# camlab-ethz/poseidon

Measured on AMD Instinct MI355X. Metric: PDE-grid samples/sec (fwd+bwd), higher is better.
Workload: dtype fp16

## Files before the change

### poseidon_amd/csrc/block_fused.h

```cpp
#pragma once
#include "common.h"

template <int C> struct KPitch { static constexpr int KP = (C + 31) / 32 * 32, P = KP + 8; };

struct ClnRowsOut {
  const float* bias;
  void* z; int z_dt;
  float* mean; float* rstd;
  const float* time; const float* gw_w; const float* gw_b; const float* bw_w; const float* bw_b; const float* sscale;
  const float* resid;
  float* out; bf16_t* out16;
  int M, rows_per_sample;
  float eps;
};

template <int C, int TT>
__device__ __forceinline__ void cln_rows_epilogue(f32x4_t (&Y)[TT][C / 16], float* patch_base, int row0, const ClnRowsOut& p,
                                                  bf16_t* tile16 = nullptr) {
  constexpr int KJ = (C + 31) / 32, NT = C / 16, CP = C + 4;
  constexpr bool RAG = (C % 32) != 0;
  static_assert(C % 16 == 0, "channel tiles");
  const int lane = threadIdx.x & 63, wave = threadIdx.x >> 6, g = lane >> 4, lc = lane & 15;
  float* Ct = patch_base + wave * 16 * CP;
  const int prow = lane >> 2, q = lane & 3;
#pragma unroll
  for (int tt = 0; tt < TT; ++tt) {
#pragma unroll
    for (int nt = 0; nt < NT; ++nt)
#pragma unroll
      for (int r = 0; r < 4; ++r) Ct[(g * 4 + r) * CP + nt * 16 + lc] = Y[tt][nt][r];
    __builtin_amdgcn_wave_barrier();
    const int grow = row0 + tt * 16 + prow;
    const bool valid = grow < p.M;
    float v[KJ][8];
    float s1 = 0.f;
#pragma unroll
    for (int pp = 0; pp < KJ; ++pp) {
      const int col = pp * 32 + q * 8;
      const bool pv = !RAG || col < C;
#pragma unroll
      for (int j = 0; j < 8; ++j) v[pp][j] = 0.f;
      if (pv) {
        const float4 x0 = *(const float4*)(Ct + prow * CP + col), x1 = *(const float4*)(Ct + prow * CP + col + 4);
        float bb[8];
        ld8(p.bias, SCOT_F32, col, bb);
        v[pp][0] = x0.x + bb[0]; v[pp][1] = x0.y + bb[1]; v[pp][2] = x0.z + bb[2]; v[pp][3] = x0.w + bb[3];
        v[pp][4] = x1.x + bb[4]; v[pp][5] = x1.y + bb[5]; v[pp][6] = x1.z + bb[6]; v[pp][7] = x1.w + bb[7];
      }
#pragma unroll
      for (int j = 0; j < 8; ++j) s1 += v[pp][j];
    }
    s1 += __shfl_xor(s1, 1, 64); s1 += __shfl_xor(s1, 2, 64);
    const float mean = s1 * (1.0f / C);
    float s2 = 0.f;
#pragma unroll
    for (int pp = 0; pp < KJ; ++pp) {
      if (RAG && pp * 32 + q * 8 >= C) continue;
#pragma unroll
      for (int j = 0; j < 8; ++j) { const float d = v[pp][j] - mean; s2 += d * d; }
    }
    s2 += __shfl_xor(s2, 1, 64); s2 += __shfl_xor(s2, 2, 64);
    const float rstd = 1.0f / sqrtf(s2 * (1.0f / C) + p.eps);
    if (valid) {
      const size_t base = (size_t)grow * C;
      if (p.mean && q == 0) { p.mean[grow] = mean; p.rstd[grow] = rstd; }
      const int samp = grow / p.rows_per_sample;
      const float t = p.time ? p.time[samp] : 0.f;
      const float sc = p.sscale ? p.sscale[samp] : 1.f;
#pragma unroll
      for (int pp = 0; pp < KJ; ++pp) {
        const int col = pp * 32 + q * 8;
        if (RAG && col >= C) continue;
        if (p.z) st8(p.z, p.z_dt, base + col, v[pp]);
        float gw[8], gb[8], bw[8], bbv[8], res[8], o[8];
        ld8(p.gw_b, SCOT_F32, col, gb); ld8(p.bw_b, SCOT_F32, col, bbv);
        if (p.gw_w) { ld8(p.gw_w, SCOT_F32, col, gw); ld8(p.bw_w, SCOT_F32, col, bw); }
        ld8(p.resid, SCOT_F32, base + col, res);
#pragma unroll
        for (int j = 0; j < 8; ++j) {
          const float ga = p.gw_w ? gw[j] * t + gb[j] : gb[j];
          const float be = p.gw_w ? bw[j] * t + bbv[j] : bbv[j];
          o[j] = sc * (ga * ((v[pp][j] - mean) * rstd) + be) + res[j];
        }
        st8(p.out, SCOT_F32, base + col, o);
        if (p.out16) st8(p.out16, SCOT_BF16, base + col, o);
        if (tile16) store8_ct(tile16 + (tt * 16 + prow) * (C + 8) + col, o);
      }
    } else if (tile16) {
      const float zero[8] = {0.f, 0.f, 0.f, 0.f, 0.f, 0.f, 0.f, 0.f};
#pragma unroll
      for (int pp = 0; pp < KJ; ++pp)
        if (!RAG || pp * 32 + q * 8 < C) store8_ct(tile16 + (tt * 16 + prow) * (C + 8) + pp * 32 + q * 8, zero);
    }
    __builtin_amdgcn_wave_barrier();
  }
}

struct ClnRowsBwd {
  const float* g;
  const void* z; int z_dt; const float* mean; const float* rstd;
  const float* time; const float* gw_w; const float* gw_b; const float* sscale;
  bf16_t* dz;
  float* d_gw_w; float* d_gw_b; float* d_bw_w; float* d_bw_b;
  float* partial;
  int M, rows_per_sample;
};

template <int C> struct ClnBwdLds {
// ... 130 lines not shown
```

### poseidon_amd/csrc/mlp_fused.hip

```cpp
#include "common.h"
#include <stdlib.h>

#include "block_fused.h"

typedef unsigned int u32x4_t __attribute__((ext_vector_type(4)));

struct MlpArgs {
  const bf16_t* h16; const float* h;
  const bf16_t* W1; const float* b1;
  const bf16_t* W2; const float* b2;
  float* out; bf16_t* out16;
  bf16_t* act; bf16_t* dact;
  void* z; int z_dt; float* mean; float* rstd;
  const float* time; const float* gw_w; const float* gw_b; const float* bw_w; const float* bw_b; const float* sscale;
  int M, rows_per_sample, hid;
  float eps;
};

template <int C, int HC> struct MlpFwdLds {
  static constexpr size_t WBYTES = (size_t)(HC * KPitch<C>::P + C * (HC + 8)) * 2 + (size_t)256 * 4, PBYTES = (size_t)4 * 16 * (C + 4) * 4;
  static constexpr size_t bytes = WBYTES > PBYTES ? WBYTES : PBYTES;
};

template <int C, int HC, int TT, bool HTILE>
__device__ __forceinline__ void mlp_fwd_body(const MlpArgs& p, char* smem, const bf16_t* htile, bf16_t* otile = nullptr) {
  constexpr bool RAG = (C % 32) != 0;
  constexpr int KJ = (C + 31) / 32;
  constexpr int NT = C / 16;
  constexpr int NB = HC / 32;
  constexpr int P1 = KPitch<C>::P;
  constexpr int P2 = HC + 8;
  constexpr int CP = C + 4;
  constexpr int W1_EL = HC * P1, W2_EL = C * P2;
  constexpr int N1 = HC * C / 8, N2 = C * HC / 8;
  constexpr int PW1 = (N1 + 255) / 256, PW2 = (N2 + 255) / 256;
  static_assert(RAG || (N1 % 256 == 0 && N2 % 256 == 0), "weight chunk pieces must divide over the 256 threads");
  static_assert(HC <= 256 && C % 16 == 0 && HC % 32 == 0 && (W1_EL * 2) % 16 == 0 && ((W1_EL + W2_EL) * 2) % 16 == 0, "layout");
  bf16_t* W1c = (bf16_t*)smem;
  bf16_t* W2c = W1c + W1_EL;
  float* b1c = (float*)(W2c + W2_EL);

  const int tid = threadIdx.x, lane = tid & 63, wave = tid >> 6, g = lane >> 4, lc = lane & 15;
  const int HID = p.hid, nch = HID / HC;
  const int row0 = (blockIdx.x * 4 + wave) * (16 * TT);

  Frag<bf16_t> hf[TT][KJ];
#pragma unroll
  for (int tt = 0; tt < TT; ++tt) {
// ... 39 lines not shown
      *(u32x4_t*)(W1c + rho * P1 + k8) = r1[u];
    }
#pragma unroll
    for (int u = 0; u < PW2; ++u) {
      const int i = tid + u * 256;
      if (RAG && i >= N2) continue;
      const int row = i / (HC / 8), c8 = (i % (HC / 8)) * 8;
      *(u32x4_t*)(W2c + row * P2 + c8) = r2[u];
    }
    b1c[tid] = rb1;
    if (RAG) {
      constexpr int PADP = (KPitch<C>::KP - C) / 8;
      const u32x4_t z = {0u, 0u, 0u, 0u};
      for (int i = tid; i < HC * PADP; i += 256) *(u32x4_t*)(W1c + (i / PADP) * P1 + C + (i % PADP) * 8) = z;
    }
  };

  f32x4_t Y[TT][NT];
#pragma unroll
  for (int tt = 0; tt < TT; ++tt)
#pragma unroll
    for (int nt = 0; nt < NT; ++nt) Y[tt][nt] = (f32x4_t){0.f, 0.f, 0.f, 0.f};

  load_chunk(0);
  store_chunk();
  __syncthreads();

  auto multiply_chunk = [&](int c) {
#pragma unroll
    for (int blk = 0; blk < NB; ++blk) {
      f32x4_t U[TT][2];
#pragma unroll
      for (int tt = 0; tt < TT; ++tt) { U[tt][0] = (f32x4_t){0.f, 0.f, 0.f, 0.f}; U[tt][1] = (f32x4_t){0.f, 0.f, 0.f, 0.f}; }
#pragma unroll
      for (int j = 0; j < KJ; ++j) {
#pragma unroll
        for (int t = 0; t < 2; ++t) {
          const Frag<bf16_t> w = lds_frag_kc(W1c, P1, blk * 32 + t * 16, j * 32, lane);
#pragma unroll
          for (int tt = 0; tt < TT; ++tt) mma16(U[tt][t], w, hf[tt][j]);
        }
      }
      const float4 ba = *(const float4*)(b1c + blk * 32 + g * 8), bb = *(const float4*)(b1c + blk * 32 + g * 8 + 4);
      const float bias[8] = {ba.x, ba.y, ba.z, ba.w, bb.x, bb.y, bb.z, bb.w};
      Frag<bf16_t> af[TT];
#pragma unroll
      for (int tt = 0; tt < TT; ++tt) {
        float av[8], dv[8];
#pragma unroll
        for (int t = 0; t < 2; ++t)
#pragma unroll
          for (int r = 0; r < 4; ++r) {
            const float x = U[tt][t][r] + bias[4 * t + r];
            float cdf, e;
            gelu_terms(x, cdf, e);
            av[4 * t + r] = x * cdf;
            dv[4 * t + r] = cdf + x * 0.3989422804014327f * e;
          }
        af[tt] = frag_from_f32<bf16_t>(av);
        if (p.act || p.dact) {
          const int row = row0 + tt * 16 + lc;
          if (row < p.M) {
            const size_t o = (size_t)row * HID + (size_t)c * HC + blk * 32 + g * 8;
            if (p.act) *(s16x8_t*)(p.act + o) = af[tt].v;
            if (p.dact) *(s16x8_t*)(p.dact + o) = frag_from_f32<bf16_t>(dv).v;
          }
        }
      }
#pragma unroll
      for (int nt = 0; nt < NT; ++nt) {
        const Frag<bf16_t> w = lds_frag_kc(W2c, P2, nt * 16, blk * 32, lane);
#pragma unroll
        for (int tt = 0; tt < TT; ++tt) mma16(Y[tt][nt], af[tt], w);
      }
    }
  };
  for (int c = 0; c + 1 < nch; ++c) {
    load_chunk(c + 1);
    multiply_chunk(c);
    __syncthreads();
    store_chunk();
    __syncthreads();
  }
  multiply_chunk(nch - 1);
  __syncthreads();

  ClnRowsOut e;
  e.bias = p.b2; e.z = p.z; e.z_dt = p.z_dt; e.mean = p.mean; e.rstd = p.rstd; e.time = p.time; e.gw_w = p.gw_w; e.gw_b = p.gw_b; e.bw_w = p.bw_w;
  e.bw_b = p.bw_b; e.sscale = p.sscale; e.resid = p.h; e.out = p.out; e.out16 = p.out16; e.M = p.M; e.rows_per_sample = p.rows_per_sample;
  e.eps = p.eps;
  cln_rows_epilogue<C, TT>(Y, (float*)smem, row0, e, otile);
}

template <int C, int HC, int TT>
__global__ __launch_bounds__(256, 2) void mlp_fused_kernel(MlpArgs p) {
  __shared__ __attribute__((aligned(16))) char smem[MlpFwdLds<C, HC>::bytes];
  mlp_fwd_body<C, HC, TT, false>(p, smem, nullptr);
}

static int mlp_chunk(int) { return 64; }

template <int C, int HC, int TT>
static int launch_mlp(const MlpArgs& a, hipStream_t s) {
  static_assert((HC * C / 8) % 256 == 0, "ragged weight chunk");
  const int rows_per_wg = 64 * TT;
  dim3 grid((a.M + rows_per_wg - 1) / rows_per_wg), block(256);
  hipLaunchKernelGGL((mlp_fused_kernel<C, HC, TT>), grid, block, 0, s, a);
  return scot_check_launch();
}

static int scot_mlp_tt_override() {
  static int tt_env = -1;
  if (tt_env < 0) { const char* e = getenv("SCOT_MLP_TT"); tt_env = e ? atoi(e) : 0; }
  return tt_env;
}

extern "C" int scot_mlp_block_fwd(const void* h16, const float* h, const void* W1, const float* b1, const void* W2, const float* b2,
                                  float* out, void* out16, void* act, void* dact, float* z, float* mean, float* rstd,
                                  const float* time, const float* gw_w, const float* gw_b, const float* bw_w, const float* bw_b,
                                  const float* sample_scale, int M, int rows_per_sample, int C, int hid, float eps,
// ... 59 lines not shown
  static constexpr size_t htile_bytes(int TT) { return (size_t)64 * TT * (C + 8) * 2; }
};

template <int C, int HC, int TT, bool KEEP, bool GIN = false, bool RECOMP = false>
__device__ __forceinline__ void mlp_bwd_body(const MlpBwdArgs& p, char* smem, float (*gkeep)[(C + 31) / 32][8],
                                             const float (*gin)[(C + 31) / 32][8] = nullptr) {
  constexpr bool RAG = (C % 32) != 0;
  constexpr int KJ = (C + 31) / 32, NT = C / 16, NB = HC / 32;
  constexpr int P1 = C + 8;
  constexpr int P2 = HC + 8;
  constexpr int CP = C + 4;
  constexpr int W1_EL = HC * P1, W2_EL = C * P2;
  constexpr int N1 = HC * C / 8, N2 = C * HC / 8;
  constexpr int PW1 = (N1 + 255) / 256, PW2 = (N2 + 255) / 256;
  static_assert((W1_EL * 2) % 16 == 0, "layout");
  static_assert(RAG || (N1 % 256 == 0 && N2 % 256 == 0), "weight chunk pieces must divide over the 256 threads");
  static_assert(!RAG || !RECOMP, "the recomputing form reads W1 K-contiguously: C % 32 == 0 only");
  bf16_t* W1c = (bf16_t*)smem;
  bf16_t* W2c = W1c + W1_EL;
  const int tid = threadIdx.x, lane = tid & 63, wave = tid >> 6, g = lane >> 4, lc = lane & 15;
  const int HID = p.hid, nch = HID / HC;
  const int wg_row0 = blockIdx.x * (64 * TT);
  const int row0 = wg_row0 + wave * (16 * TT);
  const int prow = lane >> 2, q = lane & 3;

  u32x4_t r1[PW1], r2[PW2];
  auto load_chunk = [&](int c) {
    const bf16_t* s1 = p.W1 + (size_t)c * HC * C;
#pragma unroll
    for (int u = 0; u < PW1; ++u) {
      const int i = min(tid + u * 256, N1 - 1);
      r1[u] = *(const u32x4_t*)(s1 + (size_t)i * 8);
    }
#pragma unroll
    for (int u = 0; u < PW2; ++u) {
      const int i = min(tid + u * 256, N2 - 1);
      const int row = i / (HC / 8), c8 = (i % (HC / 8)) * 8;
      r2[u] = *(const u32x4_t*)(p.W2 + (size_t)row * HID + (size_t)c * HC + c8);
    }
  };
  auto store_chunk = [&]() {
#pragma unroll
    for (int u = 0; u < PW1; ++u) {
      const int i = tid + u * 256;
      if (RAG && i >= N1) continue;
      *(u32x4_t*)(W1c + (i / (C / 8)) * P1 + (i % (C / 8)) * 8) = r1[u];
    }
// ... 115 lines not shown
        asm volatile("" ::"v"(af[tt].v));
#else
        if (p.du && rowt[tt] < p.M) *(s16x8_t*)(p.du + (size_t)rowt[tt] * HID + (size_t)c * HC + blk * 32 + g * 8) = af[tt].v;
#endif
      }
#pragma unroll
      for (int nt = 0; nt < NT; ++nt) {
        const Frag<bf16_t> w = lds_frag_ks(W1c, P1, nt * 16, blk * 32 + g * 8, blk * 32 + g * 8 + 4, lane, p.use_tr);
#pragma unroll
        for (int tt = 0; tt < TT; ++tt) mma16(Y[tt][nt], af[tt], w);
      }
    }
  };
  for (int c = 0; c + 1 < nch; ++c) {
    load_chunk(c + 1);
    multiply_chunk(c);
    __syncthreads();
    store_chunk();
    __syncthreads();
  }
  multiply_chunk(nch - 1);
  __syncthreads();

  float* Ct = (float*)smem + wave * 16 * CP;
#pragma unroll
  for (int tt = 0; tt < TT; ++tt) {
#pragma unroll
    for (int nt = 0; nt < NT; ++nt)
#pragma unroll
      for (int r = 0; r < 4; ++r) Ct[(g * 4 + r) * CP + nt * 16 + lc] = Y[tt][nt][r];
    __builtin_amdgcn_wave_barrier();
    const int grow = row0 + tt * 16 + prow;
    if (grow < p.M) {
      const size_t base = (size_t)grow * C;
#pragma unroll
      for (int pp = 0; pp < KJ; ++pp) {
        const int col = pp * 32 + q * 8;
        if (RAG && col >= C) {
          if (KEEP) {
#pragma unroll
            for (int j = 0; j < 8; ++j) gkeep[tt][pp][j] = 0.f;
          }
          continue;
        }
        const float4 x0 = *(const float4*)(Ct + prow * CP + col), x1 = *(const float4*)(Ct + prow * CP + col + 4);
        float gi[8], o[8];
        ld8(p.g, SCOT_F32, base + col, gi);
        o[0] = gi[0] + x0.x; o[1] = gi[1] + x0.y; o[2] = gi[2] + x0.z; o[3] = gi[3] + x0.w;
        o[4] = gi[4] + x1.x; o[5] = gi[5] + x1.y; o[6] = gi[6] + x1.z; o[7] = gi[7] + x1.w;
        st8(p.g_out, SCOT_F32, base + col, o);
        if (KEEP) {
#pragma unroll
          for (int j = 0; j < 8; ++j) gkeep[tt][pp][j] = o[j];
        }
      }
    } else if (KEEP) {
#pragma unroll
      for (int pp = 0; pp < KJ; ++pp)
#pragma unroll
        for (int j = 0; j < 8; ++j) gkeep[tt][pp][j] = 0.f;
    }
    __builtin_amdgcn_wave_barrier();
  }
}

template <int C, int HC, int TT>
__global__ __launch_bounds__(256, 2) void mlp_bwd_fused_kernel(MlpBwdArgs p) {
  __shared__ __attribute__((aligned(16))) char smem[MlpBwdLds<C, HC>::bytes];
  mlp_bwd_body<C, HC, TT, false>(p, smem, nullptr);
}

extern int g_scot_use_tr;
// ... 22 lines not shown
  if (rows_per_sample % 64 != 0) return SCOT_ERR_UNSUPPORTED;
  MlpBwdArgs a;
  a.g = g; a.g_out = g_out; a.z = z; a.z_dt = SCOT_F32; a.mean = mean; a.rstd = rstd; a.time = time; a.gw_w = gw_w; a.gw_b = gw_b; a.sscale = sample_scale;
  a.partial = nullptr; a.h16 = nullptr; a.b1 = nullptr;
  a.dact = (const bf16_t*)dact; a.W1 = (const bf16_t*)W1; a.W2 = (const bf16_t*)W2; a.dz = (bf16_t*)dz; a.du = (bf16_t*)du;
  a.d_gw_w = d_gw_w; a.d_gw_b = d_gw_b; a.d_bw_w = d_bw_w; a.d_bw_b = d_bw_b;
  a.M = M; a.rows_per_sample = rows_per_sample; a.hid = hid; a.use_tr = g_scot_use_tr;
  if (C == 96) {
    return tt == 2 ? launch_mlp_bwd<96, 64, 2>(a, stream) : launch_mlp_bwd<96, 64, 1>(a, stream);
  }
  return tt == 2 ? launch_mlp_bwd<192, 64, 2>(a, stream) : launch_mlp_bwd<192, 64, 1>(a, stream);
}

struct ProjClnArgs {
  const bf16_t* a; const bf16_t* W;
  ClnRowsOut e;
};

template <int C> struct ProjFwdLds {
  static constexpr size_t WBYTES = (size_t)C * (96 + 8) * 2, PBYTES = (size_t)4 * 16 * (C + 4) * 4;
  static constexpr size_t bytes = WBYTES > PBYTES ? WBYTES : PBYTES;
};

template <int C, int TT>
__device__ __forceinline__ void proj_cln_fwd_body(const ProjClnArgs& p, char* smem, bf16_t* tile16) {
  constexpr bool RAG = (C % 32) != 0;
  constexpr int KJ = (C + 31) / 32, NT = C / 16, KC = RAG ? KJ * 32 : 96, NKC = RAG ? 1 : C / KC;
  constexpr int KCR = RAG ? C : KC;
  constexpr int PW = KC + 8;
  constexpr int NP = C * KCR / 8, PWN = (NP + 255) / 256;
  static_assert(RAG || C % KC == 0, "K chunking");
  bf16_t* Wc = (bf16_t*)smem;
  const int tid = threadIdx.x, lane = tid & 63, wave = tid >> 6, g = lane >> 4, lc = lane & 15;
  const int row0 = (blockIdx.x * 4 + wave) * (16 * TT);

  Frag<bf16_t> af[TT][KJ];
#pragma unroll
  for (int tt = 0; tt < TT; ++tt) {
    const bf16_t* src = p.a + (size_t)min(row0 + tt * 16 + lc, p.e.M - 1) * C + g * 8;
    const s16x8_t zero8 = {0, 0, 0, 0, 0, 0, 0, 0};
#pragma unroll
    for (int j = 0; j < KJ; ++j) af[tt][j].v = (!RAG || j * 32 + g * 8 < C) ? *(const s16x8_t*)(src + j * 32) : zero8;
  }
  f32x4_t Y[TT][NT];
#pragma unroll
  for (int tt = 0; tt < TT; ++tt)
#pragma unroll
    for (int nt = 0; nt < NT; ++nt) Y[tt][nt] = (f32x4_t){0.f, 0.f, 0.f, 0.f};
  u32x4_t rw[PWN];
#pragma unroll
  for (int kc = 0; kc < NKC; ++kc) {
#pragma unroll
    for (int u = 0; u < PWN; ++u) {
      const int i = min(tid + u * 256, NP - 1);
      rw[u] = *(const u32x4_t*)(p.W + (size_t)(i / (KCR / 8)) * C + kc * KC + (i % (KCR / 8)) * 8);
    }
    if (kc) __syncthreads();
#pragma unroll
    for (int u = 0; u < PWN; ++u) {
      const int i = tid + u * 256;
      if (i < NP) *(u32x4_t*)(Wc + (i / (KCR / 8)) * PW + (i % (KCR / 8)) * 8) = rw[u];
    }
    if (RAG) {
      constexpr int PADP = (KC - KCR) / 8;
      const u32x4_t z = {0u, 0u, 0u, 0u};
      for (int i = tid; i < C * PADP; i += 256) *(u32x4_t*)(Wc + (i / PADP) * PW + KCR + (i % PADP) * 8) = z;
    }
    __syncthreads();
#pragma unroll
    for (int j = 0; j < KC / 32; ++j)
#pragma unroll
      for (int nt = 0; nt < NT; ++nt) {
        const Frag<bf16_t> w = lds_frag_kc(Wc, PW, nt * 16, j * 32, lane);
#pragma unroll
        for (int tt = 0; tt < TT; ++tt) mma16(Y[tt][nt], af[tt][kc * (KC / 32) + j], w);
      }
  }
  __syncthreads();
  cln_rows_epilogue<C, TT>(Y, (float*)smem, row0, p.e, tile16);
}

template <int C, int TT>
__global__ __launch_bounds__(256, 2) void proj_cln_fused_kernel(ProjClnArgs p) {
  __shared__ __attribute__((aligned(16))) char smem[ProjFwdLds<C>::bytes];
  proj_cln_fwd_body<C, TT>(p, smem, nullptr);
}

struct TailFwdArgs {
  ProjClnArgs pj; MlpArgs m;
  const bf16_t* Wqkv; const float* bqkv; bf16_t* qkv;
};

template <int C> struct QkvEpi {
  static constexpr int NC = (3 * C) % 96 == 0 ? 96 : 48;
  static constexpr size_t bytes = (size_t)NC * KPitch<C>::P * 2 + (size_t)4 * 16 * (NC + 4) * 4;
};
template <int C, int TT>
__device__ __forceinline__ void qkv_epilogue(const bf16_t* tile, const bf16_t* Wqkv, const float* bqkv, bf16_t* qkv, int M, char* smem) {
  constexpr bool RAG = (C % 32) != 0;
  constexpr int KJ = (C + 31) / 32, NC = QkvEpi<C>::NC, NCH = 3 * C / NC;
  constexpr int PW = KPitch<C>::P, NP = NC * C / 8, PWN = (NP + 255) / 256, CP = NC + 4;
  static_assert((3 * C) % NC == 0 && NC % 16 == 0, "qkv column chunks");
  const int tid = threadIdx.x, lane = tid & 63, wave = tid >> 6, g = lane >> 4, lc = lane & 15;
  const int row0 = (blockIdx.x * 4 + wave) * (16 * TT);
  Frag<bf16_t> af[TT][KJ];
#pragma unroll
  for (int tt = 0; tt < TT; ++tt)
#pragma unroll
    for (int j = 0; j < KJ; ++j) {
      const s16x8_t zero8 = {0, 0, 0, 0, 0, 0, 0, 0};
      af[tt][j].v = (!RAG || j * 32 + g * 8 < C) ? *(const s16x8_t*)(tile + (tt * 16 + lc) * (C + 8) + j * 32 + g * 8) : zero8;
    }
  bf16_t* Wc = (bf16_t*)smem;
  float* Ct = (float*)(smem + (size_t)NC * PW * 2) + wave * 16 * CP;
  const int prow = lane >> 2, q = lane & 3;
  u32x4_t rw[PWN];
#pragma unroll 1
  for (int nc = 0; nc < NCH; ++nc) {
    const bf16_t* src = Wqkv + (size_t)nc * NC * C;
#pragma unroll
    for (int u = 0; u < PWN; ++u) rw[u] = *(const u32x4_t*)(src + (size_t)min(tid + u * 256, NP - 1) * 8);
    __syncthreads();
#pragma unroll
    for (int u = 0; u < PWN; ++u) {
      const int i = tid + u * 256;
      if (i < NP) *(u32x4_t*)(Wc + (i / (C / 8)) * PW + (i % (C / 8)) * 8) = rw[u];
    }
    if (RAG) {
      constexpr int PADP = (KPitch<C>::KP - C) / 8;
      const u32x4_t z = {0u, 0u, 0u, 0u};
      for (int i = tid; i < NC * PADP; i += 256) *(u32x4_t*)(Wc + (i / PADP) * PW + C + (i % PADP) * 8) = z;
    }
    __syncthreads();
    f32x4_t Y[TT][NC / 16];
#pragma unroll
    for (int tt = 0; tt < TT; ++tt)
#pragma unroll
      for (int nt = 0; nt < NC / 16; ++nt) Y[tt][nt] = (f32x4_t){0.f, 0.f, 0.f, 0.f};
#pragma unroll
    for (int j = 0; j < KJ; ++j)
#pragma unroll
      for (int nt = 0; nt < NC / 16; ++nt) {
        const Frag<bf16_t> w = lds_frag_kc(Wc, PW, nt * 16, j * 32, lane);
#pragma unroll
        for (int tt = 0; tt < TT; ++tt) mma16(Y[tt][nt], af[tt][j], w);
      }
#pragma unroll
    for (int tt = 0; tt < TT; ++tt) {
#pragma unroll
      for (int nt = 0; nt < NC / 16; ++nt)
#pragma unroll
        for (int r = 0; r < 4; ++r) Ct[(g * 4 + r) * CP + nt * 16 + lc] = Y[tt][nt][r];
      __builtin_amdgcn_wave_barrier();
      const int grow = row0 + tt * 16 + prow;
      if (grow < M) {
#pragma unroll
        for (int pp = 0; pp < (NC + 31) / 32; ++pp) {
          const int col = pp * 32 + q * 8;
          if (NC % 32 != 0 && col >= NC) continue;
          const float4 x0 = *(const float4*)(Ct + prow * CP + col), x1 = *(const float4*)(Ct + prow * CP + col + 4);
          float o[8] = {x0.x, x0.y, x0.z, x0.w, x1.x, x1.y, x1.z, x1.w};
          if (bqkv) {
            float bb[8];
            ld8(bqkv, SCOT_F32, nc * NC + col, bb);
#pragma unroll
            for (int j = 0; j < 8; ++j) o[j] += bb[j];
          }
          st8(qkv, SCOT_BF16, (size_t)grow * (3 * C) + nc * NC + col, o);
        }
      }
      __builtin_amdgcn_wave_barrier();
    }
  }
}

template <int C, int HC, int TT, bool QKV>
__global__ __launch_bounds__(256, 2) void tail_fwd_fused_kernel(TailFwdArgs p) {
  constexpr size_t PATCH = (size_t)4 * 16 * (C + 4) * 4, TILE = (size_t)4 * 16 * TT * (C + 8) * 2;
  constexpr size_t A = ProjFwdLds<C>::bytes > PATCH + TILE ? ProjFwdLds<C>::bytes : PATCH + TILE;
  constexpr size_t QB = QkvEpi<C>::bytes;
  constexpr size_t B = A > MlpFwdLds<C, HC>::bytes ? A : MlpFwdLds<C, HC>::bytes;
  constexpr size_t LDS = (QKV && QB > B) ? QB : B;
  __shared__ __attribute__((aligned(16))) char smem[LDS];
  bf16_t* tile = (bf16_t*)(smem + PATCH) + (threadIdx.x >> 6) * 16 * TT * (C + 8);
  proj_cln_fwd_body<C, TT>(p.pj, smem, tile);
  __builtin_amdgcn_wave_barrier();
  mlp_fwd_body<C, HC, TT, true>(p.m, smem, tile, QKV ? tile : nullptr);
  if (QKV) {
    __builtin_amdgcn_wave_barrier();
    qkv_epilogue<C, TT>(tile, p.Wqkv, p.bqkv, p.qkv, p.m.M, smem);
  }
}

template <int C, int HC, int TT>
static int launch_tail_fwd(const TailFwdArgs& a, hipStream_t s) {
  dim3 grid((a.m.M + 64 * TT - 1) / (64 * TT)), block(256);
  if (a.qkv) hipLaunchKernelGGL((tail_fwd_fused_kernel<C, HC, TT, true>), grid, block, 0, s, a);
  else hipLaunchKernelGGL((tail_fwd_fused_kernel<C, HC, TT, false>), grid, block, 0, s, a);
  return scot_check_launch();
}

struct ProjClnBwdArgs {
  const bf16_t* W;
  bf16_t* da;
  ClnRowsBwd b;
  int use_tr;
};

template <int C> struct ProjBwdLds {
  static constexpr size_t WBYTES = (size_t)96 * (C + 8) * 2, PBYTES = (size_t)4 * 16 * (C + 4) * 4, P1BYTES = ClnBwdLds<C>::bytes;
  static constexpr size_t bytes = WBYTES > PBYTES ? (WBYTES > P1BYTES ? WBYTES : P1BYTES) : (PBYTES > P1BYTES ? PBYTES : P1BYTES);
};

template <int C, int TT, bool GREG>
__device__ __forceinline__ void proj_cln_bwd_body(const ProjClnBwdArgs& p, char* smem, const float (*greg)[(C + 31) / 32][8]) {
  constexpr bool RAG = (C % 32) != 0;
  constexpr int NT = C / 16, KC = RAG ? KPitch<C>::KP : 96, NKC = RAG ? 1 : C / KC;
  constexpr int KCR = RAG ? C : KC;
  constexpr int PW = C + 8;
  constexpr int NP = KCR * C / 8, PWN = (NP + 255) / 256;
  constexpr int CP = C + 4;
// ... 51 lines not shown
      for (int pp = 0; pp < (C + 31) / 32; ++pp) {
        const int col = pp * 32 + q * 8;
        if (RAG && col >= C) continue;
        const float4 x0 = *(const float4*)(Ct + prow * CP + col), x1 = *(const float4*)(Ct + prow * CP + col + 4);
        const float o[8] = {x0.x, x0.y, x0.z, x0.w, x1.x, x1.y, x1.z, x1.w};
        st8(p.da, SCOT_BF16, (size_t)grow * C + col, o);
      }
    }
    __builtin_amdgcn_wave_barrier();
  }
}

template <int C, int TT>
__global__ __launch_bounds__(256, 2) void proj_cln_bwd_fused_kernel(ProjClnBwdArgs p) {
  __shared__ __attribute__((aligned(16))) char smem[ProjBwdLds<C>::bytes];
  proj_cln_bwd_body<C, TT, false>(p, smem, nullptr);
}

struct TailBwdArgs {
  MlpBwdArgs m; ProjClnBwdArgs pj;
  const bf16_t* dqkv; const bf16_t* Wqkv;
};

template <int C, int TT>
__device__ __forceinline__ void qkv_dgrad_prologue(const bf16_t* dqkv, const bf16_t* Wqkv, float* gio, int M, char* smem, int use_tr,
                                                   float (*gk)[C / 32][8]) {
  constexpr int K3 = 3 * C, NT = C / 16, KC = 96, NKC = K3 / KC;
  constexpr int PW = C + 8, NP = KC * C / 8, PWN = (NP + 255) / 256, CP = C + 4;
  bf16_t* Wc = (bf16_t*)smem;
  const int tid = threadIdx.x, lane = tid & 63, wave = tid >> 6, g = lane >> 4, lc = lane & 15;
  const int row0 = (blockIdx.x * 4 + wave) * (16 * TT);
  f32x4_t Y[TT][NT];
#pragma unroll
  for (int tt = 0; tt < TT; ++tt)
#pragma unroll
    for (int nt = 0; nt < NT; ++nt) Y[tt][nt] = (f32x4_t){0.f, 0.f, 0.f, 0.f};
  u32x4_t rw[PWN];
#pragma unroll
  for (int kc = 0; kc < NKC; ++kc) {
    const bf16_t* src = Wqkv + (size_t)kc * KC * C;
#pragma unroll
    for (int u = 0; u < PWN; ++u) rw[u] = *(const u32x4_t*)(src + (size_t)min(tid + u * 256, NP - 1) * 8);
    Frag<bf16_t> af[TT][KC / 32];
#pragma unroll
    for (int tt = 0; tt < TT; ++tt) {
      const bf16_t* arow = dqkv + (size_t)min(row0 + tt * 16 + lc, M - 1) * K3 + kc * KC + g * 8;
#pragma unroll
// ... 4 lines not shown
    for (int u = 0; u < PWN; ++u) {
      const int i = tid + u * 256;
      if (i < NP) *(u32x4_t*)(Wc + (i / (C / 8)) * PW + (i % (C / 8)) * 8) = rw[u];
    }
    __syncthreads();
#pragma unroll
    for (int j = 0; j < KC / 32; ++j)
#pragma unroll
      for (int nt = 0; nt < NT; ++nt) {
        const Frag<bf16_t> w = lds_frag_ks(Wc, PW, nt * 16, j * 32 + g * 8, j * 32 + g * 8 + 4, lane, use_tr);
#pragma unroll
        for (int tt = 0; tt < TT; ++tt) mma16(Y[tt][nt], af[tt][j], w);
      }
  }
  __syncthreads();
  float* Ct = (float*)smem + wave * 16 * CP;
  const int prow = lane >> 2, q = lane & 3;
#pragma unroll
  for (int tt = 0; tt < TT; ++tt) {
#pragma unroll
    for (int nt = 0; nt < NT; ++nt)
#pragma unroll
      for (int r = 0; r < 4; ++r) Ct[(g * 4 + r) * CP + nt * 16 + lc] = Y[tt][nt][r];
    __builtin_amdgcn_wave_barrier();
    const int grow = row0 + tt * 16 + prow;
#pragma unroll
    for (int pp = 0; pp < C / 32; ++pp) {
      const int col = pp * 32 + q * 8;
      if (grow < M) {
        const float4 x0 = *(const float4*)(Ct + prow * CP + col), x1 = *(const float4*)(Ct + prow * CP + col + 4);
        float gi[8];
        ld8(gio, SCOT_F32, (size_t)grow * C + col, gi);
        gi[0] += x0.x; gi[1] += x0.y; gi[2] += x0.z; gi[3] += x0.w; gi[4] += x1.x; gi[5] += x1.y; gi[6] += x1.z; gi[7] += x1.w;
        st8(gio, SCOT_F32, (size_t)grow * C + col, gi);
#pragma unroll
        for (int j = 0; j < 8; ++j) gk[tt][pp][j] = gi[j];
      } else {
#pragma unroll
        for (int j = 0; j < 8; ++j) gk[tt][pp][j] = 0.f;
      }
    }
    __builtin_amdgcn_wave_barrier();
  }
}

template <int C, int HC, int TT, bool PRO, bool RECOMP>
__global__ __launch_bounds__(256, 2) void tail_bwd_fused_kernel(TailBwdArgs p) {
  constexpr size_t L0 = MlpBwdLds<C, HC>::bytes > ProjBwdLds<C>::bytes ? MlpBwdLds<C, HC>::bytes : ProjBwdLds<C>::bytes;
  constexpr size_t L1 = MlpBwdLds<C, HC>::bytes + (RECOMP ? MlpBwdLds<C, HC>::htile_bytes(TT) : 0);
  constexpr size_t LDS = L0 > L1 ? L0 : L1;
  __shared__ __attribute__((aligned(16))) char smem[LDS];
  float gk[TT][(C + 31) / 32][8];
  if constexpr (PRO) {
    static_assert(C % 32 == 0, "the qkv-dgrad prologue exists for C % 32 == 0 only");
    qkv_dgrad_prologue<C, TT>(p.dqkv, p.Wqkv, (float*)p.m.g, p.m.M, smem, p.m.use_tr, gk);
    __syncthreads();
    if (C <= 96 && !RECOMP) mlp_bwd_body<C, HC, TT, true, true, RECOMP>(p.m, smem, gk, gk);
    else mlp_bwd_body<C, HC, TT, true, false, RECOMP>(p.m, smem, gk);
  } else {
    mlp_bwd_body<C, HC, TT, true, false, RECOMP>(p.m, smem, gk);
  }
  __syncthreads();
  proj_cln_bwd_body<C, TT, true>(p.pj, smem, gk);
}

template <int C, int HC, int TT>
static int launch_tail_bwd(const TailBwdArgs& a, hipStream_t s) {
  dim3 grid((a.m.M + 64 * TT - 1) / (64 * TT)), block(256);
  if (a.m.dact == nullptr) {
    if (a.dqkv) hipLaunchKernelGGL((tail_bwd_fused_kernel<C, HC, TT, true, true>), grid, block, 0, s, a);
    else hipLaunchKernelGGL((tail_bwd_fused_kernel<C, HC, TT, false, true>), grid, block, 0, s, a);
  } else {
    if (a.dqkv) hipLaunchKernelGGL((tail_bwd_fused_kernel<C, HC, TT, true, false>), grid, block, 0, s, a);
    else hipLaunchKernelGGL((tail_bwd_fused_kernel<C, HC, TT, false, false>), grid, block, 0, s, a);
  }
  return scot_check_launch();
}

// ... 163 lines not shown
```

Measured before the change: 3540.

## Stage CLN params in LDS, prefetch residuals, and specialize tail kernels by mode

Conditional-LayerNorm parameters (bias, gamma/beta weights) are loaded once per workgroup into a small LDS region instead of per-row global loads. Residual, gradient and qkv-bias global loads are issued ahead of the LDS transpose so their latency overlaps. The tail forward kernel gets compile-time TRAIN/INFER variants, chosen on the host, that drop row bounds checks and null-pointer branches when M divides the tile. The cost is extra LDS, more live registers for the prefetched values, and more kernel instantiations.

```diff
diff --git a/poseidon_amd/csrc/block_fused.h b/poseidon_amd/csrc/block_fused.h
--- a/poseidon_amd/csrc/block_fused.h
+++ b/poseidon_amd/csrc/block_fused.h
@@ -14,24 +14,74 @@
   float eps;
 };
 
-template <int C, int TT>
-__device__ __forceinline__ void cln_rows_epilogue(f32x4_t (&Y)[TT][C / 16], float* patch_base, int row0, const ClnRowsOut& p,
-                                                  bf16_t* tile16 = nullptr) {
+enum { TAIL_GUARDED = 0, TAIL_TRAIN = 1, TAIL_INFER = 2 };
+
+template <int C> struct ClnPrm { static constexpr size_t bytes = (size_t)5 * C * 4; };
+template <int C>
+__device__ __forceinline__ void cln_params_load(const ClnRowsOut& p, float (&r)[5]) {
+  static_assert(C <= 256, "one column per thread");
+  const int c = min((int)threadIdx.x, C - 1);
+  const float* gw = p.gw_w ? p.gw_w : p.gw_b;
+  const float* bw = p.gw_w ? p.bw_w : p.bw_b;
+  r[0] = p.bias[c]; r[1] = p.gw_b[c]; r[2] = p.bw_b[c]; r[3] = gw[c]; r[4] = bw[c];
+  if (!p.gw_w) { r[3] = 0.f; r[4] = 0.f; }
+}
+template <int C>
+__device__ __forceinline__ void cln_params_store(float* prm, const float (&r)[5]) {
+  const int c = min((int)threadIdx.x, C - 1);
+#pragma unroll
+  for (int k = 0; k < 5; ++k) prm[k * C + c] = r[k];
+}
+
+template <int C, int TT, int FORM = TAIL_GUARDED, bool REQ = true>
+__device__ __forceinline__ void cln_rows_epilogue(f32x4_t (&Y)[TT][C / 16], float* patch_base, const float* prm, int row0_,
+                                                  const ClnRowsOut& p, bf16_t* tile16 = nullptr) {
+  const int row0 = __shfl_xor(row0_, 0, 64), tix = __shfl_xor((int)threadIdx.x, 0, 64);
   constexpr int KJ = (C + 31) / 32, NT = C / 16, CP = C + 4;
   constexpr bool RAG = (C % 32) != 0;
+  constexpr bool FULL = FORM != TAIL_GUARDED;
+  constexpr bool AHEAD = TT * KJ <= 6;
+  constexpr int RT = AHEAD ? TT : 1;
   static_assert(C % 16 == 0, "channel tiles");
-  const int lane = threadIdx.x & 63, wave = threadIdx.x >> 6, g = lane >> 4, lc = lane & 15;
+  const int lane = tix & 63, wave = tix >> 6, g = lane >> 4, lc = lane & 15;
   float* Ct = patch_base + wave * 16 * CP;
   const int prow = lane >> 2, q = lane & 3;
+  float res[RT][KJ][8], tv[RT], scv[RT];
+  auto request = [&](int tt, int slot) {
+    const int grow = row0 + tt * 16 + prow;
+    const int rowc = FULL ? grow : min(grow, p.M - 1);
+    const size_t base = (size_t)rowc * C;
+#pragma unroll
+    for (int pp = 0; pp < KJ; ++pp)
+      if (!RAG || pp * 32 + q * 8 < C) ld8(p.resid, SCOT_F32, base + pp * 32 + q * 8, res[slot][pp]);
+    const int samp = rowc / p.rows_per_sample;
+    tv[slot] = p.time ? p.time[samp] : 0.f;
+    scv[slot] = p.sscale ? p.sscale[samp] : 1.f;
+  };
+  auto lds8 = [&](const float* s, float (&o)[8]) {
+    const float4 a = *(const float4*)s, b = *(const float4*)(s + 4);
+    o[0] = a.x; o[1] = a.y; o[2] = a.z; o[3] = a.w; o[4] = b.x; o[5] = b.y; o[6] = b.z; o[7] = b.w;
+  };
 #pragma unroll
   for (int tt = 0; tt < TT; ++tt) {
+    const int slot = AHEAD ? tt : 0;
 #pragma unroll
     for (int nt = 0; nt < NT; ++nt)
 #pragma unroll
       for (int r = 0; r < 4; ++r) Ct[(g * 4 + r) * CP + nt * 16 + lc] = Y[tt][nt][r];
     __builtin_amdgcn_wave_barrier();
+    if (!REQ) {
+      tv[0] = scv[0] = 0.f;
+    } else if (AHEAD) {
+      if (tt == 0) {
+#pragma unroll
+        for (int t2 = 0; t2 < TT; ++t2) request(t2, t2);
+      }
+    } else {
+      request(tt, 0);
+    }
     const int grow = row0 + tt * 16 + prow;
-    const bool valid = grow < p.M;
+    const bool valid = FULL || grow < p.M;
     float v[KJ][8];
     float s1 = 0.f;
 #pragma unroll
@@ -43,7 +93,7 @@
       if (pv) {
         const float4 x0 = *(const float4*)(Ct + prow * CP + col), x1 = *(const float4*)(Ct + prow * CP + col + 4);
         float bb[8];
-        ld8(p.bias, SCOT_F32, col, bb);
+        lds8(prm + col, bb);
         v[pp][0] = x0.x + bb[0]; v[pp][1] = x0.y + bb[1]; v[pp][2] = x0.z + bb[2]; v[pp][3] = x0.w + bb[3];
         v[pp][4] = x1.x + bb[4]; v[pp][5] = x1.y + bb[5]; v[pp][6] = x1.z + bb[6]; v[pp][7] = x1.w + bb[7];
       }
@@ -56,6 +106,7 @@
 #pragma unroll
     for (int pp = 0; pp < KJ; ++pp) {
       if (RAG && pp * 32 + q * 8 >= C) continue;
+      __builtin_amdgcn_sched_barrier(0);
 #pragma unroll
       for (int j = 0; j < 8; ++j) { const float d = v[pp][j] - mean; s2 += d * d; }
     }
@@ -63,27 +114,33 @@
     const float rstd = 1.0f / sqrtf(s2 * (1.0f / C) + p.eps);
     if (valid) {
       const size_t base = (size_t)grow * C;
-      if (p.mean && q == 0) { p.mean[grow] = mean; p.rstd[grow] = rstd; }
-      const int samp = grow / p.rows_per_sample;
-      const float t = p.time ? p.time[samp] : 0.f;
-      const float sc = p.sscale ? p.sscale[samp] : 1.f;
+      if (FORM == TAIL_TRAIN) { p.mean[grow] = mean; p.rstd[grow] = rstd; }
+      else if (FORM == TAIL_GUARDED && p.mean && q == 0) { p.mean[grow] = mean; p.rstd[grow] = rstd; }
+      float t = tv[slot], sc = scv[slot];
+      if (!REQ) {
+        const int samp = grow / p.rows_per_sample;
+        t = p.time ? p.time[samp] : 0.f;
+        sc = p.sscale ? p.sscale[samp] : 1.f;
+      }
+      const bool cond = p.gw_w != nullptr;
 #pragma unroll
       for (int pp = 0; pp < KJ; ++pp) {
         const int col = pp * 32 + q * 8;
         if (RAG && col >= C) continue;
-        if (p.z) st8(p.z, p.z_dt, base + col, v[pp]);
-        float gw[8], gb[8], bw[8], bbv[8], res[8], o[8];
-        ld8(p.gw_b, SCOT_F32, col, gb); ld8(p.bw_b, SCOT_F32, col, bbv);
-        if (p.gw_w) { ld8(p.gw_w, SCOT_F32, col, gw); ld8(p.bw_w, SCOT_F32, col, bw); }
-        ld8(p.resid, SCOT_F32, base + col, res);
+        __builtin_amdgcn_sched_barrier(0);
+        if (FORM == TAIL_TRAIN) st8(p.z, SCOT_BF16, base + col, v[pp]);
+        else if (FORM == TAIL_GUARDED && p.z) st8(p.z, p.z_dt, base + col, v[pp]);
+        float gw[8], gb[8], bw[8], bbv[8], o[8];
+        lds8(prm + C + col, gb); lds8(prm + 2 * C + col, bbv); lds8(prm + 3 * C + col, gw); lds8(prm + 4 * C + col, bw);
+        if (!REQ) ld8(p.resid, SCOT_F32, base + col, res[slot][pp]);
 #pragma unroll
         for (int j = 0; j < 8; ++j) {
-          const float ga = p.gw_w ? gw[j] * t + gb[j] : gb[j];
-          const float be = p.gw_w ? bw[j] * t + bbv[j] : bbv[j];
-          o[j] = sc * (ga * ((v[pp][j] - mean) * rstd) + be) + res[j];
+          const float ga = cond ? gw[j] * t + gb[j] : gb[j];
+          const float be = cond ? bw[j] * t + bbv[j] : bbv[j];
+          o[j] = sc * (ga * ((v[pp][j] - mean) * rstd) + be) + res[slot][pp][j];
         }
         st8(p.out, SCOT_F32, base + col, o);
-        if (p.out16) st8(p.out16, SCOT_BF16, base + col, o);
+        if (FULL || p.out16) st8(p.out16, SCOT_BF16, base + col, o);
         if (tile16) store8_ct(tile16 + (tt * 16 + prow) * (C + 8) + col, o);
       }
     } else if (tile16) {
diff --git a/poseidon_amd/csrc/mlp_fused.hip b/poseidon_amd/csrc/mlp_fused.hip
--- a/poseidon_amd/csrc/mlp_fused.hip
+++ b/poseidon_amd/csrc/mlp_fused.hip
@@ -22,8 +22,8 @@
   static constexpr size_t bytes = WBYTES > PBYTES ? WBYTES : PBYTES;
 };
 
-template <int C, int HC, int TT, bool HTILE>
-__device__ __forceinline__ void mlp_fwd_body(const MlpArgs& p, char* smem, const bf16_t* htile, bf16_t* otile = nullptr) {
+template <int C, int HC, int TT, bool HTILE, int FORM = TAIL_GUARDED>
+__device__ __forceinline__ void mlp_fwd_body(const MlpArgs& p, char* smem, float* prm, const bf16_t* htile, bf16_t* otile = nullptr) {
   constexpr bool RAG = (C % 32) != 0;
   constexpr int KJ = (C + 31) / 32;
   constexpr int NT = C / 16;
@@ -109,8 +109,17 @@
 #pragma unroll
     for (int nt = 0; nt < NT; ++nt) Y[tt][nt] = (f32x4_t){0.f, 0.f, 0.f, 0.f};
 
-  load_chunk(0);
-  store_chunk();
+  ClnRowsOut e;
+  e.bias = p.b2; e.z = p.z; e.z_dt = p.z_dt; e.mean = p.mean; e.rstd = p.rstd; e.time = p.time; e.gw_w = p.gw_w; e.gw_b = p.gw_b; e.bw_w = p.bw_w;
+  e.bw_b = p.bw_b; e.sscale = p.sscale; e.resid = p.h; e.out = p.out; e.out16 = p.out16; e.M = p.M; e.rows_per_sample = p.rows_per_sample;
+  e.eps = p.eps;
+  {
+    float pr[5];
+    cln_params_load<C>(e, pr);
+    load_chunk(0);
+    store_chunk();
+    cln_params_store<C>(prm, pr);
+  }
   __syncthreads();
 
   auto multiply_chunk = [&](int c) {
@@ -145,7 +154,9 @@
             dv[4 * t + r] = cdf + x * 0.3989422804014327f * e;
           }
         af[tt] = frag_from_f32<bf16_t>(av);
-        if (p.act || p.dact) {
+        if (FORM == TAIL_TRAIN) {
+          *(s16x8_t*)(p.dact + (size_t)(row0 + tt * 16 + lc) * HID + (size_t)c * HC + blk * 32 + g * 8) = frag_from_f32<bf16_t>(dv).v;
+        } else if (FORM == TAIL_GUARDED && (p.act || p.dact)) {
           const int row = row0 + tt * 16 + lc;
           if (row < p.M) {
             const size_t o = (size_t)row * HID + (size_t)c * HC + blk * 32 + g * 8;
@@ -172,17 +183,13 @@
   multiply_chunk(nch - 1);
   __syncthreads();
 
-  ClnRowsOut e;
-  e.bias = p.b2; e.z = p.z; e.z_dt = p.z_dt; e.mean = p.mean; e.rstd = p.rstd; e.time = p.time; e.gw_w = p.gw_w; e.gw_b = p.gw_b; e.bw_w = p.bw_w;
-  e.bw_b = p.bw_b; e.sscale = p.sscale; e.resid = p.h; e.out = p.out; e.out16 = p.out16; e.M = p.M; e.rows_per_sample = p.rows_per_sample;
-  e.eps = p.eps;
-  cln_rows_epilogue<C, TT>(Y, (float*)smem, row0, e, otile);
+  cln_rows_epilogue<C, TT, FORM>(Y, (float*)smem, prm, row0, e, otile);
 }
 
 template <int C, int HC, int TT>
 __global__ __launch_bounds__(256, 2) void mlp_fused_kernel(MlpArgs p) {
-  __shared__ __attribute__((aligned(16))) char smem[MlpFwdLds<C, HC>::bytes];
-  mlp_fwd_body<C, HC, TT, false>(p, smem, nullptr);
+  __shared__ __attribute__((aligned(16))) char smem[MlpFwdLds<C, HC>::bytes + ClnPrm<C>::bytes];
+  mlp_fwd_body<C, HC, TT, false>(p, smem, (float*)(smem + MlpFwdLds<C, HC>::bytes), nullptr);
 }
 
 static int mlp_chunk(int) { return 64; }
@@ -288,7 +295,6 @@
   const int HID = p.hid, nch = HID / HC;
   const int wg_row0 = blockIdx.x * (64 * TT);
   const int row0 = wg_row0 + wave * (16 * TT);
-  const int prow = lane >> 2, q = lane & 3;
 
   u32x4_t r1[PW1], r2[PW2];
   auto load_chunk = [&](int c) {
@@ -450,17 +456,25 @@
   multiply_chunk(nch - 1);
   __syncthreads();
 
-  float* Ct = (float*)smem + wave * 16 * CP;
+  const int tid3 = RECOMP ? tid : __shfl_xor(tid, 0, 64), lane3 = tid3 & 63, wave3 = tid3 >> 6, g3 = lane3 >> 4, lc3 = lane3 & 15;
+  const int prow = lane3 >> 2, q = lane3 & 3, row3 = wg_row0 + wave3 * (16 * TT);
+  float* Ct = (float*)smem + wave3 * 16 * CP;
 #pragma unroll
   for (int tt = 0; tt < TT; ++tt) {
 #pragma unroll
     for (int nt = 0; nt < NT; ++nt)
 #pragma unroll
-      for (int r = 0; r < 4; ++r) Ct[(g * 4 + r) * CP + nt * 16 + lc] = Y[tt][nt][r];
+      for (int r = 0; r < 4; ++r) Ct[(g3 * 4 + r) * CP + nt * 16 + lc3] = Y[tt][nt][r];
+    const int grow = row3 + tt * 16 + prow;
+    const size_t base = (size_t)grow * C;
+    float gi[KJ][8];
+    if (!RECOMP && grow < p.M) {
+#pragma unroll
+      for (int pp = 0; pp < KJ; ++pp)
+        if (!RAG || pp * 32 + q * 8 < C) ld8(p.g, SCOT_F32, base + pp * 32 + q * 8, gi[pp]);
+    }
     __builtin_amdgcn_wave_barrier();
-    const int grow = row0 + tt * 16 + prow;
     if (grow < p.M) {
-      const size_t base = (size_t)grow * C;
 #pragma unroll
       for (int pp = 0; pp < KJ; ++pp) {
         const int col = pp * 32 + q * 8;
@@ -472,10 +486,10 @@
           continue;
         }
         const float4 x0 = *(const float4*)(Ct + prow * CP + col), x1 = *(const float4*)(Ct + prow * CP + col + 4);
-        float gi[8], o[8];
-        ld8(p.g, SCOT_F32, base + col, gi);
-        o[0] = gi[0] + x0.x; o[1] = gi[1] + x0.y; o[2] = gi[2] + x0.z; o[3] = gi[3] + x0.w;
-        o[4] = gi[4] + x1.x; o[5] = gi[5] + x1.y; o[6] = gi[6] + x1.z; o[7] = gi[7] + x1.w;
+        float o[8];
+        if (RECOMP) ld8(p.g, SCOT_F32, base + col, gi[pp]);
+        o[0] = gi[pp][0] + x0.x; o[1] = gi[pp][1] + x0.y; o[2] = gi[pp][2] + x0.z; o[3] = gi[pp][3] + x0.w;
+        o[4] = gi[pp][4] + x1.x; o[5] = gi[pp][5] + x1.y; o[6] = gi[pp][6] + x1.z; o[7] = gi[pp][7] + x1.w;
         st8(p.g_out, SCOT_F32, base + col, o);
         if (KEEP) {
 #pragma unroll
@@ -544,8 +558,8 @@
   static constexpr size_t bytes = WBYTES > PBYTES ? WBYTES : PBYTES;
 };
 
-template <int C, int TT>
-__device__ __forceinline__ void proj_cln_fwd_body(const ProjClnArgs& p, char* smem, bf16_t* tile16) {
+template <int C, int TT, int FORM = TAIL_GUARDED, bool REQ = true>
+__device__ __forceinline__ void proj_cln_fwd_body(const ProjClnArgs& p, char* smem, float* prm, bf16_t* tile16) {
   constexpr bool RAG = (C % 32) != 0;
   constexpr int KJ = (C + 31) / 32, NT = C / 16, KC = RAG ? KJ * 32 : 96, NKC = RAG ? 1 : C / KC;
   constexpr int KCR = RAG ? C : KC;
@@ -555,6 +569,8 @@
   bf16_t* Wc = (bf16_t*)smem;
   const int tid = threadIdx.x, lane = tid & 63, wave = tid >> 6, g = lane >> 4, lc = lane & 15;
   const int row0 = (blockIdx.x * 4 + wave) * (16 * TT);
+  float pr[5];
+  cln_params_load<C>(p.e, pr);
 
   Frag<bf16_t> af[TT][KJ];
 #pragma unroll
@@ -598,14 +614,15 @@
         for (int tt = 0; tt < TT; ++tt) mma16(Y[tt][nt], af[tt][kc * (KC / 32) + j], w);
       }
   }
+  cln_params_store<C>(prm, pr);
   __syncthreads();
-  cln_rows_epilogue<C, TT>(Y, (float*)smem, row0, p.e, tile16);
+  cln_rows_epilogue<C, TT, FORM, REQ>(Y, (float*)smem, prm, row0, p.e, tile16);
 }
 
 template <int C, int TT>
 __global__ __launch_bounds__(256, 2) void proj_cln_fused_kernel(ProjClnArgs p) {
-  __shared__ __attribute__((aligned(16))) char smem[ProjFwdLds<C>::bytes];
-  proj_cln_fwd_body<C, TT>(p, smem, nullptr);
+  __shared__ __attribute__((aligned(16))) char smem[ProjFwdLds<C>::bytes + ClnPrm<C>::bytes];
+  proj_cln_fwd_body<C, TT, TAIL_GUARDED, C != 192>(p, smem, (float*)(smem + ProjFwdLds<C>::bytes), nullptr);
 }
 
 struct TailFwdArgs {
@@ -617,13 +634,13 @@
   static constexpr int NC = (3 * C) % 96 == 0 ? 96 : 48;
   static constexpr size_t bytes = (size_t)NC * KPitch<C>::P * 2 + (size_t)4 * 16 * (NC + 4) * 4;
 };
-template <int C, int TT>
+template <int C, int TT, bool FULL>
 __device__ __forceinline__ void qkv_epilogue(const bf16_t* tile, const bf16_t* Wqkv, const float* bqkv, bf16_t* qkv, int M, char* smem) {
   constexpr bool RAG = (C % 32) != 0;
   constexpr int KJ = (C + 31) / 32, NC = QkvEpi<C>::NC, NCH = 3 * C / NC;
   constexpr int PW = KPitch<C>::P, NP = NC * C / 8, PWN = (NP + 255) / 256, CP = NC + 4;
   static_assert((3 * C) % NC == 0 && NC % 16 == 0, "qkv column chunks");
-  const int tid = threadIdx.x, lane = tid & 63, wave = tid >> 6, g = lane >> 4, lc = lane & 15;
+  const int tid = __shfl_xor((int)threadIdx.x, 0, 64), lane = tid & 63, wave = tid >> 6, g = lane >> 4, lc = lane & 15;
   const int row0 = (blockIdx.x * 4 + wave) * (16 * TT);
   Frag<bf16_t> af[TT][KJ];
 #pragma unroll
@@ -642,6 +659,11 @@
     const bf16_t* src = Wqkv + (size_t)nc * NC * C;
 #pragma unroll
     for (int u = 0; u < PWN; ++u) rw[u] = *(const u32x4_t*)(src + (size_t)min(tid + u * 256, NP - 1) * 8);
+    float bq[(NC + 31) / 32][8];
+    const float* bsrc = bqkv ? bqkv + nc * NC : (const float*)Wqkv;
+#pragma unroll
+    for (int pp = 0; pp < (NC + 31) / 32; ++pp)
+      if (NC % 32 == 0 || pp * 32 + q * 8 < NC) ld8(bsrc, SCOT_F32, pp * 32 + q * 8, bq[pp]);
     __syncthreads();
 #pragma unroll
     for (int u = 0; u < PWN; ++u) {
@@ -675,7 +697,7 @@
         for (int r = 0; r < 4; ++r) Ct[(g * 4 + r) * CP + nt * 16 + lc] = Y[tt][nt][r];
       __builtin_amdgcn_wave_barrier();
       const int grow = row0 + tt * 16 + prow;
-      if (grow < M) {
+      if (FULL || grow < M) {
 #pragma unroll
         for (int pp = 0; pp < (NC + 31) / 32; ++pp) {
           const int col = pp * 32 + q * 8;
@@ -683,10 +705,8 @@
           const float4 x0 = *(const float4*)(Ct + prow * CP + col), x1 = *(const float4*)(Ct + prow * CP + col + 4);
           float o[8] = {x0.x, x0.y, x0.z, x0.w, x1.x, x1.y, x1.z, x1.w};
           if (bqkv) {
-            float bb[8];
-            ld8(bqkv, SCOT_F32, nc * NC + col, bb);
-#pragma unroll
-            for (int j = 0; j < 8; ++j) o[j] += bb[j];
+#pragma unroll
+            for (int j = 0; j < 8; ++j) o[j] += bq[pp][j];
           }
           st8(qkv, SCOT_BF16, (size_t)grow * (3 * C) + nc * NC + col, o);
         }
@@ -696,29 +716,50 @@
   }
 }
 
-template <int C, int HC, int TT, bool QKV>
+template <int C, int HC, int TT, bool QKV, int FORM>
 __global__ __launch_bounds__(256, 2) void tail_fwd_fused_kernel(TailFwdArgs p) {
   constexpr size_t PATCH = (size_t)4 * 16 * (C + 4) * 4, TILE = (size_t)4 * 16 * TT * (C + 8) * 2;
   constexpr size_t A = ProjFwdLds<C>::bytes > PATCH + TILE ? ProjFwdLds<C>::bytes : PATCH + TILE;
   constexpr size_t QB = QkvEpi<C>::bytes;
   constexpr size_t B = A > MlpFwdLds<C, HC>::bytes ? A : MlpFwdLds<C, HC>::bytes;
   constexpr size_t LDS = (QKV && QB > B) ? QB : B;
-  __shared__ __attribute__((aligned(16))) char smem[LDS];
+  static_assert(LDS % 16 == 0, "the parameter rows follow");
+  __shared__ __attribute__((aligned(16))) char smem[LDS + ClnPrm<C>::bytes];
   bf16_t* tile = (bf16_t*)(smem + PATCH) + (threadIdx.x >> 6) * 16 * TT * (C + 8);
-  proj_cln_fwd_body<C, TT>(p.pj, smem, tile);
+  float* prm = (float*)(smem + LDS);
+  proj_cln_fwd_body<C, TT, FORM>(p.pj, smem, prm, tile);
   __builtin_amdgcn_wave_barrier();
-  mlp_fwd_body<C, HC, TT, true>(p.m, smem, tile, QKV ? tile : nullptr);
+  mlp_fwd_body<C, HC, TT, true, FORM>(p.m, smem, prm, tile, QKV ? tile : nullptr);
   if (QKV) {
     __builtin_amdgcn_wave_barrier();
-    qkv_epilogue<C, TT>(tile, p.Wqkv, p.bqkv, p.qkv, p.m.M, smem);
+    qkv_epilogue<C, TT, FORM != TAIL_GUARDED>(tile, p.Wqkv, p.bqkv, p.qkv, p.m.M, smem);
+  }
+}
+
+static int tail_form(const TailFwdArgs& a, int rows_per_wg) {
+  const MlpArgs& m = a.m;
+  const ClnRowsOut& e = a.pj.e;
+  if (m.M % rows_per_wg != 0 || !m.out16 || !e.out16 || m.act) return TAIL_GUARDED;
+  const bool all = e.z && e.mean && m.z && m.mean && m.dact, none = !e.z && !e.mean && !m.z && !m.mean && !m.dact;
+  if (all && m.z_dt == SCOT_BF16 && e.z_dt == SCOT_BF16) return TAIL_TRAIN;
+  return none ? TAIL_INFER : TAIL_GUARDED;
+}
+
+template <int C, int HC, int TT, bool QKV>
+static void launch_tail_fwd_form(const TailFwdArgs& a, dim3 grid, hipStream_t s) {
+  const dim3 block(256);
+  switch (tail_form(a, 64 * TT)) {
+    case TAIL_TRAIN: hipLaunchKernelGGL((tail_fwd_fused_kernel<C, HC, TT, QKV, TAIL_TRAIN>), grid, block, 0, s, a); break;
+    case TAIL_INFER: hipLaunchKernelGGL((tail_fwd_fused_kernel<C, HC, TT, QKV, TAIL_INFER>), grid, block, 0, s, a); break;
+    default: hipLaunchKernelGGL((tail_fwd_fused_kernel<C, HC, TT, QKV, TAIL_GUARDED>), grid, block, 0, s, a);
   }
 }
 
 template <int C, int HC, int TT>
 static int launch_tail_fwd(const TailFwdArgs& a, hipStream_t s) {
-  dim3 grid((a.m.M + 64 * TT - 1) / (64 * TT)), block(256);
-  if (a.qkv) hipLaunchKernelGGL((tail_fwd_fused_kernel<C, HC, TT, true>), grid, block, 0, s, a);
-  else hipLaunchKernelGGL((tail_fwd_fused_kernel<C, HC, TT, false>), grid, block, 0, s, a);
+  dim3 grid((a.m.M + 64 * TT - 1) / (64 * TT));
+  if (a.qkv) launch_tail_fwd_form<C, HC, TT, true>(a, grid, s);
+  else launch_tail_fwd_form<C, HC, TT, false>(a, grid, s);
   return scot_check_launch();
 }
 
@@ -816,7 +857,7 @@
   const bf16_t* dqkv; const bf16_t* Wqkv;
 };
 
-template <int C, int TT>
+template <int C, int TT, bool AHEAD>
 __device__ __forceinline__ void qkv_dgrad_prologue(const bf16_t* dqkv, const bf16_t* Wqkv, float* gio, int M, char* smem, int use_tr,
                                                    float (*gk)[C / 32][8]) {
   constexpr int K3 = 3 * C, NT = C / 16, KC = 96, NKC = K3 / KC;
@@ -867,15 +908,20 @@
     for (int nt = 0; nt < NT; ++nt)
 #pragma unroll
       for (int r = 0; r < 4; ++r) Ct[(g * 4 + r) * CP + nt * 16 + lc] = Y[tt][nt][r];
+    const int grow = row0 + tt * 16 + prow;
+    float gin[C / 32][8];
+    if (AHEAD && grow < M) {
+#pragma unroll
+      for (int pp = 0; pp < C / 32; ++pp) ld8(gio, SCOT_F32, (size_t)grow * C + pp * 32 + q * 8, gin[pp]);
+    }
     __builtin_amdgcn_wave_barrier();
-    const int grow = row0 + tt * 16 + prow;
 #pragma unroll
     for (int pp = 0; pp < C / 32; ++pp) {
       const int col = pp * 32 + q * 8;
       if (grow < M) {
         const float4 x0 = *(const float4*)(Ct + prow * CP + col), x1 = *(const float4*)(Ct + prow * CP + col + 4);
-        float gi[8];
-        ld8(gio, SCOT_F32, (size_t)grow * C + col, gi);
+        float (&gi)[8] = gin[pp];
+        if (!AHEAD) ld8(gio, SCOT_F32, (size_t)grow * C + col, gi);
         gi[0] += x0.x; gi[1] += x0.y; gi[2] += x0.z; gi[3] += x0.w; gi[4] += x1.x; gi[5] += x1.y; gi[6] += x1.z; gi[7] += x1.w;
         st8(gio, SCOT_F32, (size_t)grow * C + col, gi);
 #pragma unroll
@@ -898,7 +944,7 @@
   float gk[TT][(C + 31) / 32][8];
   if constexpr (PRO) {
     static_assert(C % 32 == 0, "the qkv-dgrad prologue exists for C % 32 == 0 only");
-    qkv_dgrad_prologue<C, TT>(p.dqkv, p.Wqkv, (float*)p.m.g, p.m.M, smem, p.m.use_tr, gk);
+    qkv_dgrad_prologue<C, TT, !RECOMP>(p.dqkv, p.Wqkv, (float*)p.m.g, p.m.M, smem, p.m.use_tr, gk);
     __syncthreads();
     if (C <= 96 && !RECOMP) mlp_bwd_body<C, HC, TT, true, true, RECOMP>(p.m, smem, gk, gk);
     else mlp_bwd_body<C, HC, TT, true, false, RECOMP>(p.m, smem, gk);
```

Measured after the change: 3575, median of 6. Within noise of the previous version (+1.0%).
